# jgsimard/big-dreamer

Measured on AMD Instinct MI355X. Metric: latent transitions/sec (RSSM + imagination) at batch=50 chunk=50 H=15, higher is better.
Workload: dtype f32

## Files before the change

big_dreamer_amd/_cabi.py:

```python
from __future__ import annotations

import ctypes as C
import os

import torch

_HERE = os.path.dirname(os.path.abspath(__file__))
LIB_PATH = os.environ.get("BD_LIB") or os.path.join(_HERE, "libbigdreamer_hip.so")

if not os.path.exists(LIB_PATH):
    raise ImportError(
        f"{LIB_PATH} is missing: the MI355X HIP extension has not been built "
        "(run `python -c 'import __graft_entry__ as g; g.build()'`). There is no CPU fallback.")

lib = C.CDLL(LIB_PATH)

BD_MAX_LAYERS = 6
ACT_NONE, ACT_ELU, ACT_ELU_GRAD = 0, 1, 2
ACT_RELU, ACT_RELU_GRAD, ACT_TANH, ACT_TANH_GRAD = 3, 4, 5, 6
CNN_ACTS = {"ELU": (ACT_ELU, ACT_ELU_GRAD), "ReLU": (ACT_RELU, ACT_RELU_GRAD), "Tanh": (ACT_TANH, ACT_TANH_GRAD)}
GRAD_ACTS = (ACT_ELU_GRAD, ACT_RELU_GRAD, ACT_TANH_GRAD)
P = C.c_void_p
F32 = C.c_float
I32 = C.c_int
# ... 8 lines not shown


class MlpFwdArgs(C.Structure):
    _fields_ = [("M", I32), ("in0", P), ("ld0", I32), ("w0", I32), ("in1", P), ("ld1", I32), ("w1", I32),
                ("n_layers", I32), ("layer", Layer * BD_MAX_LAYERS), ("out", P), ("ldo", I32),
                ("gidx", P), ("gWT", P), ("gD", I32), ("gC", I32)]


class LayerBwd(C.Structure):
    _fields_ = [("wt", P), ("saved", P), ("N", I32), ("K", I32), ("act", I32), ("dpre", P)]


class MlpBwdArgs(C.Structure):
    _fields_ = [("M", I32), ("dout", P), ("lddo", I32), ("dout_scale", F32), ("n_layers", I32),
                ("layer", LayerBwd * BD_MAX_LAYERS), ("din0", P), ("ld0", I32), ("w0", I32),
                ("din1", P), ("ld1", I32), ("w1", I32), ("accumulate", I32), ("form_M", I32)]


BD_HEAD_HIDDEN = 4


class ImgHead(C.Structure):
    _fields_ = [("w", P * BD_HEAD_HIDDEN), ("wt", P * BD_HEAD_HIDDEN), ("b", P * BD_HEAD_HIDDEN),
                ("w_out", P), ("b_out", P), ("dout", P), ("out", P)]


class ImgHeadsArgs(C.Structure):
    _fields_ = [("M", I32), ("F", I32), ("Hd", I32), ("x", P), ("head", ImgHead * 2), ("dx", P)]


BD_RNG_MAX_TENSORS = 6
BD_RNG_NORMAL, BD_RNG_EXPONENTIAL, BD_RNG_UNIFORM = 0, 1, 2


class RngTensor(C.Structure):
    _fields_ = [("p", P), ("count", C.c_size_t), ("kind", I32), ("stream_id", C.c_uint)]


class RngFillArgs(C.Structure):
    _fields_ = [("n", I32), ("seed", C.c_ulonglong), ("step", C.c_ulonglong), ("t", RngTensor * BD_RNG_MAX_TENSORS)]


class WgradDesc(C.Structure):
# ... 170 lines not shown
    "bd_gemm_nt": (I32, [P, I32, P, I32, P, I32, I32, I32, I32, I32, P]),
    "bd_categorical_head_forward": (I32, [P, P, I32, I32, I32, P, P, P]),
    "bd_categorical_head_backward": (I32, [P, P, I32, I32, I32, P, P]),
    "bd_kl_categorical_forward": (I32, [P, P, I32, I32, I32, F32, I32, P, I32, P, P]),
    "bd_kl_categorical_backward": (I32, [P, P, I32, I32, I32, F32, F32, F32, F32, P, I32, P, P, P]),
    "bd_plan_rollout": (I32, [C.POINTER(PlanArgs), P]),
    "bd_cem_refit": (I32, [P, I32, P, I32, I32, I32, I32, I32, P, P, P]),
    "bd_plan_rollout_cat": (I32, [C.POINTER(PlanCatArgs), P]),
    "bd_act_step_supported": (I32, [I32, I32, I32, I32, I32, I32]),
    "bd_act_step": (I32, [C.POINTER(ActArgs), P]),
    "bd_act_step_cat_supported": (I32, [I32] * 10),
    "bd_act_step_cat": (I32, [C.POINTER(ActCatArgs), P]),
    "bd_lambda_return_backward": (I32, [P, F32, I32, I32, F32, F32, P, P, P]),
    "bd_img_heads_supported": (I32, [I32, I32]),
    "bd_img_heads_fwd_bwd": (I32, [C.POINTER(ImgHeadsArgs), P]),
    "bd_actor_reinforce": (I32, [P, P, P, P, P, P, P, I32, I32, I32, F32, F32, F32, I32, P, P, I32, P, P]),
    "bd_actor_reinforce_cat": (I32, [P, P, P, P, P, P, I32, I32, I32, F32, F32, F32, I32, P, P, I32, P, P]),
    "bd_normal_nll": (I32, [P, I32, P, I32, I32, I32, F32, P, I32, P, I32, P, P]),
    "bd_bernoulli_nll": (I32, [P, P, C.c_size_t, F32, P, P, I32, P, P]),
    "bd_kl_forward": (I32, [P, P, P, P, I32, I32, F32, I32, P, I32, P, P]),
    "bd_kl_backward": (I32, [P, P, P, P, I32, I32, F32, F32, F32, F32, P, I32, P, P, P, P, P]),
    "bd_sum": (I32, [P, C.c_size_t, P, I32, P, P]),
    "bd_sumsq": (I32, [P, C.c_size_t, P, I32, P, P]),
    "bd_adam_step": (I32, [P, P, P, P, C.c_size_t, F32, F32, F32, F32, F32, I32, F32, P, I32, P]),
    "bd_polyak": (I32, [P, P, C.c_size_t, F32, P]),
    "bd_replay_gather": (I32, [P, P, I32, I32, P, P]),
    "bd_replay_gather_pixels": (I32, [P, P, I32, I32, I32, P, P, P]),
    "bd_replay_gather_pixels_rng": (I32, [P, P, I32, I32, I32, C.c_ulonglong, C.c_ulonglong, P, P]),
    "bd_replay_append": (I32, [C.POINTER(ReplayAppendArgs), P]),
    "bd_reduce_ws_floats": (C.c_size_t, []),
# ... 45 lines not shown
```

big_dreamer_amd/csrc/mlp.hip:

```cpp
#include "bd_device.h"
#include "bd_host.h"
#include <stdlib.h>

namespace bd {

template <bool ANY>
__device__ __forceinline__ floatx4 chain_act4(int act, floatx4 x) {
    if constexpr (ANY) return act_apply4(act, x);
    floatx4 v = x;
    if (act) {
#pragma unroll
        for (int r = 0; r < 4; ++r) v[r] = elu(x[r]);
    }
    return v;
}
template <bool ANY>
__device__ __forceinline__ float chain_grad(int act, float y) {
    if constexpr (ANY) return act_grad_from_out(act, y);
    return elu_grad_from_out(y);
}

template <int RT, bool ANY>
__global__ __launch_bounds__(kThreads) void mlp_fwd_kernel(bd_mlp_fwd_args a, int KbA, int KbB) {
    extern __shared__ __attribute__((aligned(16))) float smem[];
// ... 130 lines not shown
        float* t = cur; cur = nxt; nxt = t;
    }
    if (a.din0 != nullptr || a.din1 != nullptr) {
        const bd_layer_bwd L = a.layer[0];
        const Seg segs[1] = {{cur, L.wt, cdiv(L.N, 16)}};
        tile_linear_pre<RT, 1, true>(segs, nullptr, L.K, NoPre{}, [&](int rt, int nb, floatx4 acc, NoPreVal) {
            const int ln = bd_tid() & 63, col0 = nb * 16 + 4 * (ln >> 4);
            const int grow = row0 + rt * 16 + (ln & 15);
            if (grow >= a.M) return;
#pragma unroll
            for (int r = 0; r < 4; ++r) {
                const int col = col0 + r;
                float* p = nullptr;
                if (col < a.w0) { if (a.din0) p = a.din0 + (size_t)grow * a.ld0 + col; }
                else if (col < a.w0 + a.w1) { if (a.din1) p = a.din1 + (size_t)grow * a.ld1 + (col - a.w0); }
                if (p) *p = a.accumulate ? *p + acc[r] : acc[r];
            }
        }, scratch);
    }
}

#ifdef BD_STAMPS
__device__ unsigned long long g_tallstamps[64];
#define TALL_STAMP(slot)                                                                                         \
    do {                                                                                                         \
        if (blockIdx.x == 0 && threadIdx.x == 0 && (slot) < 64) g_tallstamps[slot] = __builtin_amdgcn_s_memtime(); \
    } while (0)
#else
#define TALL_STAMP(slot)
#endif

template <int RT, bool ANY>
__global__ __launch_bounds__(kThreads) __attribute__((amdgpu_waves_per_eu(3, 3))) void mlp_fwd_tall_kernel(bd_mlp_fwd_args a) {
// ... 270 lines not shown
    bool any = false;
    for (int l = a->n_layers - 1, j = 0; l >= 0; --l, ++j) {
        const bd_layer_bwd& L = a->layer[l];
        any = any || (L.act != BD_ACT_NONE && L.act != BD_ACT_ELU);
        BD_REQUIRE(L.N > 0 && L.K > 0, "bd_mlp_backward: layer %d has bad dims", l);
        BD_REQUIRE(L.act == BD_ACT_NONE || act_is_forward(L.act), "bd_mlp_backward: layer %d has unknown activation code %d", l, L.act);
        BD_REQUIRE(!L.act || L.saved, "bd_mlp_backward: layer %d needs its saved output", l);
        BD_REQUIRE(l == 0 ? (!want_din || L.wt) : (L.wt != nullptr), "bd_mlp_backward: layer %d needs packed W^T", l);
        BD_REQUIRE(l == 0 || a->layer[l - 1].N == L.K, "bd_mlp_backward: layer %d K mismatch", l);
        int& kb = (j & 1) ? KbB : KbA;
        kb = cdiv(L.N, 16) > kb ? cdiv(L.N, 16) : kb;
    }
    if (want_din) BD_REQUIRE(a->w0 + a->w1 == a->layer[0].K, "bd_mlp_backward: din widths != K of layer 0");
    BD_REQUIRE(a->form_M >= 0, "bd_mlp_backward: bad form_M");
    const int Mf = a->form_M > 0 ? a->form_M : a->M;
    if (tall_enabled() && cdiv(Mf, 16) >= (tall_mode == 2 ? 1 : kTallMinTiles)) {
        bool ok = true;
        size_t widest = (size_t)(a->ld0 > a->ld1 ? a->ld0 : a->ld1);
        auto al16 = [](const void* q) { return (reinterpret_cast<uintptr_t>(q) & 15) == 0; };
        for (int l = a->n_layers - 1; l >= 1; --l) {
            const bd_layer_bwd& P = a->layer[l - 1];
            ok = ok && tall_shape_ok(a->layer[l].K, kTallRT) && (P.N & 3) == 0 && al16(P.saved) && al16(P.dpre);
            widest = (size_t)a->layer[l].K > widest ? (size_t)a->layer[l].K : widest;
        }
        ok = ok && (size_t)a->M * widest < ((size_t)1 << 31);
        int kb = KbA > KbB ? KbA : KbB;
        if (want_din) kb = cdiv(a->layer[0].N, 16) > kb ? cdiv(a->layer[0].N, 16) : kb;
        if (ok && any) return launch_tall(mlp_bwd_tall_kernel<kTallRT, true>, "bd_mlp_backward(tall)", a->M, kb, (hipStream_t)stream, *a);
        if (ok) return launch_tall(mlp_bwd_tall_kernel<kTallRT, false>, "bd_mlp_backward(tall)", a->M, kb, (hipStream_t)stream, *a);
    }
    const int rt = pick_rt(Mf, KbA, KbB);
    if (any) {
        if (rt == 2) return launch_chain(mlp_bwd_kernel<2, true>, "bd_mlp_backward", a->M, 2, KbA, KbB, (hipStream_t)stream, *a);
        return launch_chain(mlp_bwd_kernel<1, true>, "bd_mlp_backward", a->M, 1, KbA, KbB, (hipStream_t)stream, *a);
    }
    if (rt == 2) return launch_chain(mlp_bwd_kernel<2, false>, "bd_mlp_backward", a->M, 2, KbA, KbB, (hipStream_t)stream, *a);
    return launch_chain(mlp_bwd_kernel<1, false>, "bd_mlp_backward", a->M, 1, KbA, KbB, (hipStream_t)stream, *a);
}

}
```

big_dreamer_amd/engine.py:

```python
from __future__ import annotations

import collections.abc
import ctypes as C
import math
import os
import weakref
from typing import Dict, List, Optional, Tuple

import numpy as np
import torch

from . import _cabi as cabi
from .parallel import DataParallel
from .params import ParamGroup, _adam_state_dict, _load_adam_state_dict
from .synth import CNN_ACTIVATIONS, DENSE_LAYERS, MODEL_MODULES, Dims, model_modules, param_shapes

lib = cabi.lib
ptr = cabi.ptr

DEFAULT_HP = dict(
    kl_balance=0.8, kl_loss_weight=0.1, free_nats=3.0, grad_clip_norm=100.0, discount=0.995, disclam=0.95,
    model_learning_rate=2e-4, actor_learning_rate=4e-5, value_learning_rate=1e-4, adam_epsilon=1e-5,
    weight_decay=1e-6, entropy_weight=1e-5, polyak_avg=1.0, min_std_dev=0.1, discount_weight=5.0,
    gradient_mixing=-1,
# ... 193 lines not shown
        self._mod_group.update(actor="actor", critic="critic", critic_target="critic_target")
        if params is not None:
            self.load_params(params)
        self.scalars = torch.zeros(N_SLOTS, dtype=torch.float32, device=self.dev)
        self.red_ws = torch.zeros(int(lib.bd_reduce_ws_floats()), dtype=torch.float32, device=self.dev)
        self._wgrad_ws = torch.zeros(1, dtype=torch.float32, device=self.dev)
        self._wgrad_ws_side = torch.zeros(1, dtype=torch.float32, device=self.dev)
        self._wgrad_ws_early = torch.zeros(1, dtype=torch.float32, device=self.dev)
        self.red_ws_side = torch.zeros(int(lib.bd_reduce_ws_floats()), dtype=torch.float32, device=self.dev)
        self._wbatch = {"model": WgradBatch(self, "model"), "model_early": WgradBatch(self, "model_early", "_wgrad_ws_early"),
                        "actor": WgradBatch(self, "actor", "_wgrad_ws_bh"),
                        "critic": WgradBatch(self, "critic", "_wgrad_ws_side")}
        self._side = _engine_stream(self.dev, "side", int(os.environ.get("BD_SIDE_PRIO", "0")))
        self.heads_fused = (os.environ.get("BD_HEADS_FUSED", "1") != "0" and not self.d.categorical
                            and bool(lib.bd_img_heads_supported(self.d.Be + self.d.S, self.d.Hd)))
        self._s_early = _engine_stream(self.dev, "early", int(os.environ.get("BD_EARLY_PRIO", "0")))
        self.bh_chunks = _parse_bh_chunks(os.environ.get("BD_BH_CHUNKS", ""))
        self.bh_chunks_bwd = os.environ.get("BD_BH_CHUNKS_BWD", "0") == "1"
        self._s_ov = self._side
        self.pipeline = os.environ.get("BD_PIPELINE", "1") != "0"
        self._s_wm = _engine_stream(self.dev, "wm", int(os.environ.get("BD_WM_PRIO", "-1")))
        bh_prio = int(os.environ.get("BD_BH_PRIO", "0" if self.pixel else "-1"))
        self._s_bh = _engine_stream(self.dev, "bh", bh_prio)
        self._ev_bh_wm_free: Optional[torch.cuda.Event] = None
        self._bh_plan_used: Optional[Tuple[int, ...]] = None
        self._ev_bh_done: List[Optional[torch.cuda.Event]] = [None, None]
        self._ev_cr_done: List[Optional[torch.cuda.Event]] = [None, None]
        shared_comm = not all(g in self.dp.groups for g in ("model", "actor", "critic"))
        self.defer_opt = (world_size > 1 and shared_comm) or os.environ.get("BD_DEFER_OPT", "0") == "1"
        if os.environ.get("BD_FORCE_DP", "0") == "1" and torch.distributed.is_initialized():
# ... 215 lines not shown
    def mlp_forward(self, M, in0, ld0, w0, layers, saves, out, ldo, in1=None, ld1=0, w1=0, raw_packs=False,
                    gather=None) -> None:
        a = cabi.MlpFwdArgs()
        a.M, a.in0, a.ld0, a.w0 = M, ptr(in0), ld0, w0
        a.in1, a.ld1, a.w1 = ptr(in1), ld1, w1
        if gather is not None:
            a.gidx, a.gWT, a.gD, a.gC = ptr(gather[0]), ptr(gather[1]), gather[2], gather[3]
        a.n_layers = len(layers)
        for i, (key, bias, N, K, act) in enumerate(layers):
            a.layer[i] = cabi.Layer(ptr(key if raw_packs else self.pk[key]), ptr(bias), N, K, act,
                                    ptr(saves[i]) if saves else None)
        a.out, a.ldo = ptr(out), ldo
        cabi.check(lib.bd_mlp_forward(C.byref(a), cabi.stream()))

    def mlp_backward(self, M, dout, lddo, layers, saves, dpres, din0=None, ld0=0, w0=0, din1=None, ld1=0, w1=0,
                     accumulate=False, dout_scale=1.0, raw_packs=False, form_M=0) -> None:
        a = cabi.MlpBwdArgs()
        a.M, a.dout, a.lddo, a.dout_scale, a.form_M = M, ptr(dout), lddo, dout_scale, form_M
        a.n_layers = len(layers)
        for i, (key, _bias, N, K, act) in enumerate(layers):
            wt = key if raw_packs else self.pk.get(key + ".T")
            a.layer[i] = cabi.LayerBwd(ptr(wt) if wt is not None else None,
                                       ptr(saves[i]) if (saves and saves[i] is not None) else None, N, K, act,
                                       ptr(dpres[i]) if (dpres and dpres[i] is not None) else None)
        a.din0, a.ld0, a.w0 = ptr(din0), ld0, w0
        a.din1, a.ld1, a.w1 = ptr(din1), ld1, w1
        a.accumulate = int(accumulate)
        cabi.check(lib.bd_mlp_backward(C.byref(a), cabi.stream()))

    def wgrad(self, dpre, ldp, act, lda, M, N, K, dW, ldw, db=None, accumulate=False) -> None:
        need = int(lib.bd_wgrad_ws_floats(M, N, K))
        if self._wgrad_ws.numel() < need:
            self._wgrad_ws = torch.zeros(need, dtype=torch.float32, device=self.dev)
        cabi.check(lib.bd_wgrad(ptr(dpre), ldp, ptr(act), lda, M, N, K, ptr(dW), ldw, ptr(db), int(accumulate),
                                ptr(self._wgrad_ws), self._wgrad_ws.numel(), cabi.stream()))

    def _dense_wgrads(self, batch: "WgradBatch", mod: str, M: int, dpres, inp, ld_in, saves, sizes) -> None:
        for l in range(len(sizes) - 1):
            act, lda = (inp, ld_in) if l == 0 else (saves[l - 1], sizes[l])
            batch.add(dpres[l], sizes[l + 1], act, lda, M, sizes[l + 1], sizes[l],
                      self.G(mod, f"model.{2 * l}.weight"), sizes[l], self.G(mod, f"model.{2 * l}.bias"))

# ... 703 lines not shown
        N = T * B
        F = d.Be + d.S
        W = self.world_size
        st = cabi.stream()
        sc, ws = ptr(self.scalars), ptr(self.red_ws)

        obs_t = obs[1:].reshape(N, d.O)
        with self.span("encoder_fwd"):
            emb, pre_emb = self.encode_pixels(obs[1:].reshape(N, 3, 64, 64)) if self.pixel else self.encode(obs_t, N)
        init_belief = self.buf("init_belief", B, d.Be).zero_()
        init_state = self.buf("init_state", B, d.S).zero_()
        feat, qm, qs = self.observe(actions[:-1], nonterm[:-1], pre_emb, noise["obs_post"], init_belief, init_state, T, B,
                                    feat_tag=feat_tag)
        cat = d.categorical
        sidx = self._buf[feat_tag + "sidx"] if cat else None
        with self.span("wm_heads_fwd"):
            _, pm, ps = self.prior_head(feat, N, None if cat else noise.get("obs_prior"))
            if self.pixel:
                om_out, om_acts, om_layers = self.conv.decode(feat).view(N, d.O), None, None
                obs_t = self.conv.acts_enc[0].view(N, d.O)
            else:
                om_out, om_acts, om_layers = self.dense_forward("observation_model", "obs", "om", feat, F, N, d.O,
                                                                sidx=sidx)
            rw_out, rw_acts, rw_layers = self.dense_forward("reward_model", "rew", "rw", feat, F, N, 1, sidx=sidx)

        inv_rows = self.dp.mean_grad_scale(N)
        dc_state = None
        if d.use_discount:
            dc_out, dc_acts, dc_layers = self.dense_forward("discount_model", "dsc", "dc", feat, F, N, 1, sidx=sidx)
            d_dc = self.buf("d_dc_out", N, 1)
            cabi.check(lib.bd_bernoulli_nll(ptr(dc_out), ptr(nonterm[:-1]), N, hp["discount_weight"] * inv_rows, ptr(d_dc), sc,
                                            SLOT_DISC, ws, st))
            dc_state = (d_dc, dc_acts, dc_layers)
        d_om, d_rw = self.buf("d_om_out", N, d.O), self.buf("d_rw_out", N, 1)
        cabi.check(lib.bd_normal_nll(ptr(om_out), d.O, ptr(obs_t), d.O, N, d.O, inv_rows, ptr(d_om), d.O, sc, SLOT_OBS, ws, st))
        cabi.check(lib.bd_normal_nll(ptr(rw_out), 1, ptr(rewards[:-1]), 1, N, 1, inv_rows, ptr(d_rw), 1, sc, SLOT_REW, ws, st))
        sum_form = int(hp["kl_balance"] == -1)
        kl_n = d.cat_D if cat else d.S
        if cat:
            cabi.check(lib.bd_kl_categorical_forward(ptr(qm), ptr(pm), N, d.cat_D, d.cat_C, hp["free_nats"], sum_form, sc,
                                                     SLOT_KL, ws, st))
        else:
            cabi.check(lib.bd_kl_forward(ptr(qm), ptr(qs), ptr(pm), ptr(ps), N, d.S, hp["free_nats"], sum_form, sc, SLOT_KL,
                                         ws, st))
        if W > 1 and not sum_form:
            self._kl_local = self.scalars[SLOT_KL:SLOT_KL + 1].clone()
            self._allreduce(self.scalars[SLOT_KL:SLOT_KL + 1], "model")
        kl_inv = 1.0 / (N * kl_n * W) if not sum_form else 1.0 / (N * W)
        kl_w = hp["kl_loss_weight"] * (1.0 / W if sum_form else 1.0)
        if cat:
            dqm, dpm = self.buf("dql", N, d.S), self.buf("dpl", N, d.S)
            cabi.check(lib.bd_kl_categorical_backward(ptr(qm), ptr(pm), N, d.cat_D, d.cat_C, hp["free_nats"], hp["kl_balance"],
                                                      kl_w, kl_inv, sc, SLOT_KL, ptr(dqm), ptr(dpm), st))
        else:
            dqm, dqs = self.buf("dqm", N, d.S), self.buf("dqs", N, d.S)
            dpm, dps = self.buf("dpm", N, d.S), self.buf("dps", N, d.S)
            cabi.check(lib.bd_kl_backward(ptr(qm), ptr(qs), ptr(pm), ptr(ps), N, d.S, hp["free_nats"], hp["kl_balance"],
                                          kl_w, kl_inv, sc, SLOT_KL, ptr(dqm), ptr(dqs), ptr(dpm), ptr(dps), st))

        dfeat = self.buf("dfeat", N, F)
        rw_dpre = [self.buf(f"rw_dpre{l}", N, d.Hd) for l in range(DENSE_LAYERS)] + [d_rw]
        if self.pixel:
            self.mlp_backward(N, d_rw, 1, rw_layers, rw_acts + [None], rw_dpre[:-1] + [None], din0=dfeat, ld0=F, w0=F)
            with self.span("decoder_bwd"):
                self.conv.backward_decoder(d_om.view(N, 64, 64, 3), feat, dfeat, self._wbatch["model_early"])
                self._s_early.wait_stream(torch.cuda.current_stream())
                with torch.cuda.stream(self._s_early):
                    self._wbatch["model_early"].run()
        else:
            om_dpre = [self.buf(f"om_dpre{l}", N, d.Hd) for l in range(DENSE_LAYERS)] + [d_om]
            self.mlp_backward(N, d_om, d.O, om_layers, om_acts + [None], om_dpre[:-1] + [None], din0=dfeat, ld0=F, w0=F)
            self.mlp_backward(N, d_rw, 1, rw_layers, rw_acts + [None], rw_dpre[:-1] + [None], din0=dfeat, ld0=F, w0=F,
                              accumulate=True)
        dc_dpre = None
        if dc_state is not None:
            d_dc, dc_acts, dc_layers = dc_state
            dc_dpre = [self.buf(f"dc_dpre{l}", N, d.Hd) for l in range(DENSE_LAYERS)] + [d_dc]
            self.mlp_backward(N, d_dc, 1, dc_layers, dc_acts + [None], dc_dpre[:-1] + [None], din0=dfeat, ld0=F, w0=F,
                              accumulate=True)
        self._dc_wgrad = (dc_dpre, dc_state[1]) if dc_state is not None else None
        p_out, p_hid = self._buf["p_out"], self._buf["p_hid"]
        HO = d.head_out
        d_p_hid = self.buf("d_p_hid", N, d.Hd)
        if cat:
            d_p_out = dpm
        else:
            d_p_out = self.buf("d_p_out", N, HO)
            cabi.check(lib.bd_gauss_head_backward(ptr(p_out), None, None, ptr(dpm), ptr(dps), N, d.S, ptr(d_p_out), st))
        p_layers = [("p1", None, d.Hd, d.Be, cabi.ACT_ELU), ("p2", None, HO, d.Hd, cabi.ACT_NONE)]
        self.mlp_backward(N, d_p_out, HO, p_layers, [p_hid, None], [d_p_hid, None], din0=dfeat, ld0=F, w0=d.Be,
                          accumulate=True)
        d_e, d_gi, d_gh, d_q1, d_q2 = self._observe_backward(T, B, nonterm[:-1], noise["obs_post"], feat)
        self._dynamics_tail(batch, emb, obs_t, feat, init_belief, actions, d_e, d_gi, d_gh, d_q1, d_q2, d_p_hid, d_p_out,
                            p_hid, rw_dpre, rw_acts, om_dpre if (not self.pixel) else None,
                            om_acts if (not self.pixel) else None, N, B, F)
        return feat

    def _observe_backward(self, T: int, B: int, nonterm, eps_post, feat):
        d, pk, buf = self.d, self.pk, self._buf
        N = T * B
        if d.categorical:
            b = cabi.ObserveCatBwdArgs()
            b.D, b.C = d.cat_D, d.cat_C
            b.wt_q2 = ptr(pk["q2.T"])
            b.post_logits, b.dpost_logits = ptr(buf["post_logits"]), ptr(buf["dql"])
            scan, scan_cluster = lib.bd_observe_cat_backward, lib.bd_observe_cat_backward_cluster
# ... 51 lines not shown
        dense_sizes = lambda i, o: [i] + [d.Hd] * DENSE_LAYERS + [o]
        self._dense_wgrads(wb, "reward_model", N, rw_dpre, feat, F, rw_acts, dense_sizes(F, 1))
        if self._dc_wgrad is not None:
            self._dense_wgrads(wb, "discount_model", N, self._dc_wgrad[0], feat, F, self._dc_wgrad[1], dense_sizes(F, 1))
        if not self.pixel:
            self._dense_wgrads(wb, "observation_model", N, om_dpre, feat, F, om_acts, dense_sizes(F, d.O))
            self._dense_wgrads(wb, "encoder", N, enc_dpre, obs_t, d.O, enc_acts, dense_sizes(d.O, d.E))
        with self.span("wgrad_model"):
            wb.run()
        if self.pixel:
            torch.cuda.current_stream().wait_stream(self._s_early)
        if self.pipeline and self._ev_bh_wm_free is not None:
            torch.cuda.current_stream().wait_event(self._ev_bh_wm_free)
        with self.span("opt_model"):
            self.optimizer_step("model", SLOT_GN_MODEL, hp["model_learning_rate"])

    def img_heads_fused(self, M: int, x, d_r, d_v, r_out, v_out, dx) -> None:
        d = self.d
        a = cabi.ImgHeadsArgs()
        a.M, a.F, a.Hd, a.x, a.dx = M, d.Be + d.S, d.Hd, ptr(x), ptr(dx)
        for h, (mod, prefix, dout, out) in enumerate((("reward_model", "rew", d_r, r_out),
                                                      ("critic_target", "tgt", d_v, v_out))):
            H = a.head[h]
            for l in range(DENSE_LAYERS):
                H.w[l], H.wt[l] = ptr(self.pk[f"{prefix}{l}"]), ptr(self.pk[f"{prefix}{l}.T"])
                H.b[l] = ptr(self.W(mod, f"model.{2 * l}.bias"))
            H.w_out = ptr(self.W(mod, f"model.{2 * DENSE_LAYERS}.weight"))
            H.b_out = ptr(self.W(mod, f"model.{2 * DENSE_LAYERS}.bias"))
            H.dout, H.out = ptr(dout), ptr(out)
        cabi.check(lib.bd_img_heads_fwd_bwd(C.byref(a), cabi.stream()))
# ... 293 lines not shown
```

include/bigdreamer_hip.h:

```cpp
#ifndef BIGDREAMER_HIP_H
#define BIGDREAMER_HIP_H

#include <stddef.h>
#include <stdint.h>

#ifdef __cplusplus
extern "C" {
#endif

#define BD_MAX_LAYERS 6
#define BD_ACT_NONE 0
#define BD_ACT_ELU 1
#define BD_ACT_ELU_GRAD 2
#define BD_ACT_RELU 3
#define BD_ACT_RELU_GRAD 4
#define BD_ACT_TANH 5
#define BD_ACT_TANH_GRAD 6

const char* bd_last_error(void);
int bd_version(void);

typedef struct {
    const float* src;
    float* dst;
// ... 30 lines not shown
    int N, K;
    int act;
    float* dpre;
} bd_layer_bwd;

typedef struct {
    int M;
    const float* dout; int lddo;
    float dout_scale;
    int n_layers;
    bd_layer_bwd layer[BD_MAX_LAYERS];
    float* din0; int ld0, w0;
    float* din1; int ld1, w1;
    int accumulate;
    int form_M;
} bd_mlp_bwd_args;
int bd_mlp_backward(const bd_mlp_bwd_args* a, void* stream);

int bd_mlp_set_tall(int mode);

size_t bd_wgrad_ws_floats(int M, int N, int K);
int bd_wgrad(const float* dpre, int ldp, const float* act, int lda, int M, int N, int K,
             float* dW, int ldw, float* db, int accumulate, float* ws, size_t ws_floats, void* stream);

typedef struct {
    const float* dpre; int ldp;
    const float* act1; int lda1; int M1;
    const float* act2; int lda2;
    int M, N, K;
    float* dW; int ldw;
// ... 166 lines not shown
    const float* wt[BD_HEAD_HIDDEN];
    const float* b[BD_HEAD_HIDDEN];
    const float* w_out;
    const float* b_out;
    const float* dout;
    float* out;
} bd_img_head;
typedef struct {
    int M, F, Hd;
    const float* x;
    bd_img_head head[2];
    float* dx;
} bd_img_heads_args;
int bd_img_heads_supported(int F, int Hd);
int bd_img_heads_fwd_bwd(const bd_img_heads_args* a, void* stream);

int bd_actor_reinforce(const float* eps_action, const float* act_us, const float* act_stats, const float* returns,
                       const float* base0, const float* value, const float* weight, int Hm, int N, int A, float rho,
                       float grad_scale, float dentropy, int write, float* d_actor_out, float* scalars, int slot, float* ws,
                       void* stream);
int bd_actor_reinforce_cat(const float* action, const float* act_stats, const float* returns, const float* base0,
                           const float* value, const float* weight, int Hm, int N, int A, float rho, float grad_scale,
                           float dentropy, int write, float* d_actor_out, float* scalars, int slot, float* ws,
                           void* stream);

#define BD_RNG_MAX_TENSORS 6
#define BD_RNG_NORMAL 0
#define BD_RNG_EXPONENTIAL 1
#define BD_RNG_UNIFORM 2
typedef struct {
// ... 246 lines not shown
```

Before: 13.46 million.

## Fuse world-model obs, reward and prior heads into one forward+backward kernel

Adds a wm_heads kernel that runs the observation and reward decoder MLPs (forward, loss gradient, backward to the input) and the belief prior head (forward and Gaussian parameterisation) as three block-row chains in a single launch, keeping activations in LDS. The reward head's input gradient goes to a side buffer and is folded into dfeat by a new din0_add path in the next accumulating mlp_backward, replacing separate forward, NLL-gradient and backward launches. This cuts launches and round-trips of activations through global memory. In exchange it adds LDS pressure, only 16-row tiles per block, and a constraint that the tall backward form cannot take the add path.

```diff
diff --git a/big_dreamer_amd/_cabi.py b/big_dreamer_amd/_cabi.py
--- a/big_dreamer_amd/_cabi.py
+++ b/big_dreamer_amd/_cabi.py
@@ -46,7 +46,8 @@
 class MlpBwdArgs(C.Structure):
     _fields_ = [("M", I32), ("dout", P), ("lddo", I32), ("dout_scale", F32), ("n_layers", I32),
                 ("layer", LayerBwd * BD_MAX_LAYERS), ("din0", P), ("ld0", I32), ("w0", I32),
-                ("din1", P), ("ld1", I32), ("w1", I32), ("accumulate", I32), ("form_M", I32)]
+                ("din1", P), ("ld1", I32), ("w1", I32), ("accumulate", I32), ("form_M", I32),
+                ("din0_add", P), ("ld_add", I32), ("w_add", I32)]
 
 
 BD_HEAD_HIDDEN = 4
@@ -59,6 +60,20 @@
 
 class ImgHeadsArgs(C.Structure):
     _fields_ = [("M", I32), ("F", I32), ("Hd", I32), ("x", P), ("head", ImgHead * 2), ("dx", P)]
+
+
+class WmLayer(C.Structure):
+    _fields_ = [("w", P), ("wt", P), ("bias", P), ("N", I32), ("K", I32), ("save", P), ("dpre", P)]
+
+
+class WmChain(C.Structure):
+    _fields_ = [("n_layers", I32), ("w_in", I32), ("layer", WmLayer * BD_MAX_LAYERS), ("out", P), ("ldo", I32),
+                ("target", P), ("ldt", I32), ("grad_scale", F32), ("dx", P), ("lddx", I32)]
+
+
+class WmHeadsArgs(C.Structure):
+    _fields_ = [("M", I32), ("S", I32), ("x", P), ("ldx", I32), ("chain", WmChain * 3), ("eps", P), ("min_std", F32),
+                ("mean", P), ("std", P), ("state", P)]
 
 
 BD_RNG_MAX_TENSORS = 6
@@ -259,6 +274,8 @@
     "bd_lambda_return_backward": (I32, [P, F32, I32, I32, F32, F32, P, P, P]),
     "bd_img_heads_supported": (I32, [I32, I32]),
     "bd_img_heads_fwd_bwd": (I32, [C.POINTER(ImgHeadsArgs), P]),
+    "bd_wm_heads_supported": (I32, [I32, I32, I32, I32, I32]),
+    "bd_wm_heads_fwd_bwd": (I32, [C.POINTER(WmHeadsArgs), P]),
     "bd_actor_reinforce": (I32, [P, P, P, P, P, P, P, I32, I32, I32, F32, F32, F32, I32, P, P, I32, P, P]),
     "bd_actor_reinforce_cat": (I32, [P, P, P, P, P, P, I32, I32, I32, F32, F32, F32, I32, P, P, I32, P, P]),
     "bd_normal_nll": (I32, [P, I32, P, I32, I32, I32, F32, P, I32, P, I32, P, P]),
diff --git a/big_dreamer_amd/csrc/mlp.hip b/big_dreamer_amd/csrc/mlp.hip
--- a/big_dreamer_amd/csrc/mlp.hip
+++ b/big_dreamer_amd/csrc/mlp.hip
@@ -168,9 +168,24 @@
                 float* p = nullptr;
                 if (col < a.w0) { if (a.din0) p = a.din0 + (size_t)grow * a.ld0 + col; }
                 else if (col < a.w0 + a.w1) { if (a.din1) p = a.din1 + (size_t)grow * a.ld1 + (col - a.w0); }
-                if (p) *p = a.accumulate ? *p + acc[r] : acc[r];
+                if (!p) continue;
+                float o = acc[r];
+                if (a.accumulate) {
+                    float b = *p;
+                    if (a.din0_add && col < a.w0) b = b + a.din0_add[(size_t)grow * a.ld_add + col];
+                    o = b + acc[r];
+                }
+                *p = o;
             }
         }, scratch);
+        if (a.din0_add && a.w_add > a.w0) {
+            const int wt = a.w_add - a.w0;
+            for (int i = bd_tid(); i < 16 * RT * wt; i += blockDim.x) {
+                const int r = i / wt, col = a.w0 + (i - r * wt);
+                const int grow = row0 + r;
+                if (grow < a.M) a.din0[(size_t)grow * a.ld0 + col] += a.din0_add[(size_t)grow * a.ld_add + col];
+            }
+        }
     }
 }
 
@@ -471,6 +486,13 @@
     if (want_din) BD_REQUIRE(a->w0 + a->w1 == a->layer[0].K, "bd_mlp_backward: din widths != K of layer 0");
     BD_REQUIRE(a->form_M >= 0, "bd_mlp_backward: bad form_M");
     const int Mf = a->form_M > 0 ? a->form_M : a->M;
+    if (a->din0_add) {
+        BD_REQUIRE(a->accumulate == 1 && a->din0, "bd_mlp_backward: din0_add needs accumulate = 1 and din0");
+        BD_REQUIRE(a->w_add == 0 || (a->w_add >= a->w0 && a->din1 == nullptr && a->ld0 >= a->w_add),
+                   "bd_mlp_backward: w_add = %d needs w0 <= w_add <= ld0 and din1 = NULL", a->w_add);
+        BD_REQUIRE(a->ld_add >= (a->w_add > a->w0 ? a->w_add : a->w0), "bd_mlp_backward: ld_add = %d is smaller than the columns added",
+                   a->ld_add);
+    }
     if (tall_enabled() && cdiv(Mf, 16) >= (tall_mode == 2 ? 1 : kTallMinTiles)) {
         bool ok = true;
         size_t widest = (size_t)(a->ld0 > a->ld1 ? a->ld0 : a->ld1);
@@ -483,6 +505,7 @@
         ok = ok && (size_t)a->M * widest < ((size_t)1 << 31);
         int kb = KbA > KbB ? KbA : KbB;
         if (want_din) kb = cdiv(a->layer[0].N, 16) > kb ? cdiv(a->layer[0].N, 16) : kb;
+        if (ok) BD_REQUIRE(!a->din0_add, "bd_mlp_backward: din0_add is not taken by the tall form (%d rows pick it)", Mf);
         if (ok && any) return launch_tall(mlp_bwd_tall_kernel<kTallRT, true>, "bd_mlp_backward(tall)", a->M, kb, (hipStream_t)stream, *a);
         if (ok) return launch_tall(mlp_bwd_tall_kernel<kTallRT, false>, "bd_mlp_backward(tall)", a->M, kb, (hipStream_t)stream, *a);
     }
diff --git a/big_dreamer_amd/csrc/wm_heads.hip b/big_dreamer_amd/csrc/wm_heads.hip
--- /dev/null
+++ b/big_dreamer_amd/csrc/wm_heads.hip
@@ -0,0 +1,234 @@
+#include "bd_device.h"
+#include "bd_host.h"
+
+namespace bd {
+
+constexpr int kWmChains = 3;
+
+template <class CL>
+__device__ __forceinline__ bd_wm_layer wm_layer(const CL& l) {
+    bd_wm_layer r;
+    r.w = l.w; r.wt = l.wt; r.bias = l.bias; r.N = l.N; r.K = l.K; r.save = l.save; r.dpre = l.dpre;
+    return r;
+}
+
+__global__ __launch_bounds__(kThreads) void wm_heads_kernel(bd_wm_heads_args a, int KbA, int KbB) {
+    extern __shared__ __attribute__((aligned(16))) float smem[];
+    BD_KARGS(bd_wm_heads_args, ka);
+    const auto& C = ka->chain[blockIdx.y];
+    const int M = ka->M, row0 = blockIdx.x * 16, n = C.n_layers;
+    const bool loss = C.target != nullptr;
+    float* cur = smem;
+    float* nxt = smem + (size_t)KbA * kFragFloats;
+    float* scratch = nxt + (size_t)KbB * kFragFloats;
+    load_tile_concat<1>(cur, cdiv(C.w_in, 16), row0, M, ka->x, ka->ldx, C.w_in, nullptr, 0, 0);
+    lds_barrier();
+    auto al16 = [](const void* q) { return (reinterpret_cast<uintptr_t>(q) & 15) == 0; };
+    for (int l = 0; l < n; ++l) {
+        const bd_wm_layer L = wm_layer(C.layer[l]);
+        const bool last = (l == n - 1);
+        const int Kb = cdiv(L.K, 16);
+        float* out = C.out;
+        const float* target = C.target;
+        const int ldo = C.ldo, ldt = C.ldt;
+        const float gs = C.grad_scale;
+        const bool vec = (L.N & 3) == 0 && (last ? (!loss && (ldo & 3) == 0 && al16(out)) : al16(L.save));
+        const Seg seg[1] = {{cur, L.w, Kb}};
+        tile_linear_pre<1, 1, true>(
+            seg, L.bias, L.N,
+            [&](int, int nb) {
+                Pre4 p;
+                const int ln = bd_tid() & 63, col0 = nb * 16 + 4 * (ln >> 4);
+                const int grow = row0 + (ln & 15);
+#pragma unroll
+                for (int r = 0; r < 4; ++r)
+                    p.v[r] = (last && loss && grow < M && col0 + r < L.N) ? target[(size_t)grow * ldt + col0 + r] : 0.f;
+                return p;
+            },
+            [&](int, int nb, floatx4 acc, const Pre4& p) {
+                const int ln = bd_tid() & 63, col0 = nb * 16 + 4 * (ln >> 4);
+                const int grow = row0 + (ln & 15);
+                floatx4 v = acc, img;
+                if (!last) {
+#pragma unroll
+                    for (int r = 0; r < 4; ++r) v[r] = elu(acc[r]);
+                }
+                img = v;
+                if (last && loss) {
+#pragma unroll
+                    for (int r = 0; r < 4; ++r) img[r] = (grow < M && col0 + r < L.N) ? (v[r] - p.v[r]) * gs : 0.f;
+                }
+                *reinterpret_cast<floatx4*>(nxt + (nb * 64 + ln) * 4) = img;
+                if (grow < M && col0 < L.N) {
+                    if (vec) {
+                        if (last) *reinterpret_cast<floatx4*>(out + (size_t)grow * ldo + col0) = v;
+                        else *reinterpret_cast<floatx4*>(L.save + (size_t)grow * L.N + col0) = v;
+                    } else {
+#pragma unroll
+                        for (int r = 0; r < 4; ++r)
+                            if (col0 + r < L.N) {
+                                if (!last) L.save[(size_t)grow * L.N + col0 + r] = v[r];
+                                else {
+                                    out[(size_t)grow * ldo + col0 + r] = v[r];
+                                    if (loss) L.dpre[(size_t)grow * L.N + col0 + r] = img[r];
+                                }
+                            }
+                    }
+                }
+            },
+            scratch);
+        if (last && loss) __syncthreads();
+        else lds_barrier();
+        float* t = cur; cur = nxt; nxt = t;
+    }
+    if (!loss) {
+        const int S = ka->S;
+        const float* eps = ka->eps;
+        const float min_std = ka->min_std;
+        float* mean = ka->mean;
+        float* std = ka->std;
+        float* state = ka->state;
+        for (int i = bd_tid(); i < 16 * S; i += kThreads) {
+            const int row = i / S, c = i - row * S;
+            const int grow = row0 + row;
+            if (grow >= M) continue;
+            const size_t g = (size_t)grow * S + c;
+            const float m = cur[frag_idx(row, c)];
+            const float sd = softplusf(cur[frag_idx(row, S + c)]) + min_std;
+            mean[g] = m;
+            std[g] = sd;
+            if (state) state[g] = m + sd * eps[g];
+        }
+        return;
+    }
+    for (int l = n - 1; l >= 1; --l) {
+        const bd_wm_layer L = wm_layer(C.layer[l]);
+        const bd_wm_layer P = wm_layer(C.layer[l - 1]);
+        const int Kb = cdiv(L.N, 16);
+        const Seg segs[1] = {{cur, L.wt, Kb}};
+        const bool vec = (P.N & 3) == 0 && al16(P.save) && al16(P.dpre);
+        tile_linear_pre<1, 1, true>(
+            segs, nullptr, L.K,
+            [&](int, int nb) {
+                Pre4 p;
+                const int ln = bd_tid() & 63, col0 = nb * 16 + 4 * (ln >> 4);
+                const int grow = row0 + (ln & 15);
+                const bool in = grow < M && col0 < P.N;
+                if (in && vec) {
+                    const floatx4 t = *reinterpret_cast<const floatx4*>(P.save + (size_t)grow * P.N + col0);
+#pragma unroll
+                    for (int r = 0; r < 4; ++r) p.v[r] = t[r];
+                } else {
+#pragma unroll
+                    for (int r = 0; r < 4; ++r) p.v[r] = (in && col0 + r < P.N) ? P.save[(size_t)grow * P.N + col0 + r] : 1.f;
+                }
+                return p;
+            },
+            [&](int, int nb, floatx4 acc, const Pre4& p) {
+                const int ln = bd_tid() & 63, col0 = nb * 16 + 4 * (ln >> 4);
+                const int grow = row0 + (ln & 15);
+                floatx4 v = floatx4{0.f, 0.f, 0.f, 0.f};
+                if (grow < M && col0 < P.N) {
+#pragma unroll
+                    for (int r = 0; r < 4; ++r)
+                        if (col0 + r < P.N) v[r] = acc[r] * elu_grad_from_out(p.v[r]);
+                    if (vec) *reinterpret_cast<floatx4*>(P.dpre + (size_t)grow * P.N + col0) = v;
+                    else {
+#pragma unroll
+                        for (int r = 0; r < 4; ++r)
+                            if (col0 + r < P.N) P.dpre[(size_t)grow * P.N + col0 + r] = v[r];
+                    }
+                }
+                *reinterpret_cast<floatx4*>(nxt + (nb * 64 + ln) * 4) = v;
+            },
+            scratch);
+        lds_barrier();
+        float* t = cur; cur = nxt; nxt = t;
+    }
+    {
+        const bd_wm_layer L = wm_layer(C.layer[0]);
+        float* dx = C.dx;
+        const int lddx = C.lddx;
+        const Seg segs[1] = {{cur, L.wt, cdiv(L.N, 16)}};
+        tile_linear_pre<1, 1, true>(segs, nullptr, L.K, NoPre{}, [&](int, int nb, floatx4 acc, NoPreVal) {
+            const int ln = bd_tid() & 63, col0 = nb * 16 + 4 * (ln >> 4);
+            const int grow = row0 + (ln & 15);
+            if (grow >= M) return;
+#pragma unroll
+            for (int r = 0; r < 4; ++r)
+                if (col0 + r < L.K) dx[(size_t)grow * lddx + col0 + r] = acc[r];
+        }, scratch);
+    }
+}
+
+static void wm_plan_chain(const int* widths, int n, bool loss, int (&cap)[2]) {
+    int b = 0;
+    auto need = [&](int w) { cap[b] = cdiv(w, 16) > cap[b] ? cdiv(w, 16) : cap[b]; };
+    need(widths[0]);
+    for (int l = 1; l <= n; ++l) { b ^= 1; need(widths[l]); }
+    if (loss)
+        for (int l = n - 1; l >= 1; --l) { b ^= 1; need(widths[l]); }
+}
+
+static size_t wm_lds(const int (&cap)[2]) {
+    return ((size_t)(cap[0] + cap[1]) * kFragFloats + kSplitScratchFloats) * sizeof(float);
+}
+
+}
+
+extern "C" {
+
+int bd_wm_heads_supported(int Be, int S, int Hd, int O, int hidden) {
+    using namespace bd;
+    if (Be <= 0 || S <= 0 || Hd <= 0 || O <= 0 || hidden < 1 || hidden + 1 > BD_MAX_LAYERS) return 0;
+    int cap[2] = {0, 0}, w[BD_MAX_LAYERS + 1];
+    w[0] = Be + S;
+    for (int l = 1; l <= hidden; ++l) w[l] = Hd;
+    w[hidden + 1] = O > 1 ? O : 1;
+    wm_plan_chain(w, hidden + 1, true, cap);
+    const int p[3] = {Be, Hd, 2 * S};
+    wm_plan_chain(p, 2, false, cap);
+    return wm_lds(cap) <= (size_t)kMaxLds;
+}
+
+int bd_wm_heads_fwd_bwd(const bd_wm_heads_args* a, void* stream) {
+    using namespace bd;
+    BD_REQUIRE(a && a->M > 0 && a->S > 0 && a->x, "bd_wm_heads_fwd_bwd: bad M / S / x");
+    BD_REQUIRE(a->mean && a->std && (!a->state || a->eps), "bd_wm_heads_fwd_bwd: the prior needs mean and std, and eps for a sample");
+    int cap[2] = {0, 0};
+    for (int c = 0; c < kWmChains; ++c) {
+        const bd_wm_chain& C = a->chain[c];
+        const bool loss = c < kWmChains - 1;
+        BD_REQUIRE(C.n_layers >= 1 && C.n_layers <= BD_MAX_LAYERS, "bd_wm_heads_fwd_bwd: chain %d has bad n_layers", c);
+        BD_REQUIRE(C.w_in > 0 && a->ldx >= C.w_in, "bd_wm_heads_fwd_bwd: chain %d reads %d columns of x (ld %d)", c, C.w_in, a->ldx);
+        int w[BD_MAX_LAYERS + 1];
+        w[0] = C.w_in;
+        for (int l = 0; l < C.n_layers; ++l) {
+            const bd_wm_layer& L = C.layer[l];
+            const bool last = l == C.n_layers - 1;
+            BD_REQUIRE(L.N > 0 && L.K == w[l], "bd_wm_heads_fwd_bwd: chain %d layer %d has K=%d, expected %d", c, l, L.K, w[l]);
+            bool ok = L.w && (last || L.save);
+            if (loss) ok = ok && L.wt && L.dpre;
+            BD_REQUIRE(ok, "bd_wm_heads_fwd_bwd: chain %d layer %d is missing an operand", c, l);
+            w[l + 1] = L.N;
+        }
+        const int Nl = w[C.n_layers];
+        BD_REQUIRE(C.out && C.ldo >= Nl, "bd_wm_heads_fwd_bwd: chain %d has a bad output", c);
+        if (loss)
+            BD_REQUIRE(C.target && C.ldt >= Nl && C.dx && C.lddx >= C.w_in,
+                       "bd_wm_heads_fwd_bwd: chain %d is missing an operand (target / dx)", c);
+        else
+            BD_REQUIRE(!C.target && Nl == 2 * a->S, "bd_wm_heads_fwd_bwd: the prior chain ends in 2S = %d columns, got %d (no target)",
+                       2 * a->S, Nl);
+        wm_plan_chain(w, C.n_layers, loss, cap);
+    }
+    const size_t lds = wm_lds(cap);
+    BD_REQUIRE(lds <= (size_t)kMaxLds, "bd_wm_heads_fwd_bwd: widths not covered: the chain images need %zu B of LDS (> %d)", lds, kMaxLds);
+    if (lds > 64 * 1024 && allow_big_lds(wm_heads_kernel)) return -1;
+    hipLaunchKernelGGL(wm_heads_kernel, dim3(cdiv(a->M, 16), kWmChains), dim3(kThreads), lds, (hipStream_t)stream, *a,
+                       cap[0], cap[1]);
+    BD_CHECK_LAUNCH("bd_wm_heads_fwd_bwd");
+    return 0;
+}
+
+}
diff --git a/big_dreamer_amd/engine.py b/big_dreamer_amd/engine.py
--- a/big_dreamer_amd/engine.py
+++ b/big_dreamer_amd/engine.py
@@ -231,6 +231,8 @@
         self._side = _engine_stream(self.dev, "side", int(os.environ.get("BD_SIDE_PRIO", "0")))
         self.heads_fused = (os.environ.get("BD_HEADS_FUSED", "1") != "0" and not self.d.categorical
                             and bool(lib.bd_img_heads_supported(self.d.Be + self.d.S, self.d.Hd)))
+        self.wm_heads_fused = (os.environ.get("BD_WM_HEADS_FUSED", "1") != "0" and not self.d.categorical and not self.pixel
+                               and bool(lib.bd_wm_heads_supported(self.d.Be, self.d.S, self.d.Hd, self.d.O, DENSE_LAYERS)))
         self._s_early = _engine_stream(self.dev, "early", int(os.environ.get("BD_EARLY_PRIO", "0")))
         self.bh_chunks = _parse_bh_chunks(os.environ.get("BD_BH_CHUNKS", ""))
         self.bh_chunks_bwd = os.environ.get("BD_BH_CHUNKS_BWD", "0") == "1"
@@ -476,7 +478,7 @@
         cabi.check(lib.bd_mlp_forward(C.byref(a), cabi.stream()))
 
     def mlp_backward(self, M, dout, lddo, layers, saves, dpres, din0=None, ld0=0, w0=0, din1=None, ld1=0, w1=0,
-                     accumulate=False, dout_scale=1.0, raw_packs=False, form_M=0) -> None:
+                     accumulate=False, dout_scale=1.0, raw_packs=False, form_M=0, din0_add=None, ld_add=0, w_add=0) -> None:
         a = cabi.MlpBwdArgs()
         a.M, a.dout, a.lddo, a.dout_scale, a.form_M = M, ptr(dout), lddo, dout_scale, form_M
         a.n_layers = len(layers)
@@ -488,6 +490,7 @@
         a.din0, a.ld0, a.w0 = ptr(din0), ld0, w0
         a.din1, a.ld1, a.w1 = ptr(din1), ld1, w1
         a.accumulate = int(accumulate)
+        a.din0_add, a.ld_add, a.w_add = ptr(din0_add), ld_add, w_add
         cabi.check(lib.bd_mlp_backward(C.byref(a), cabi.stream()))
 
     def wgrad(self, dpre, ldp, act, lda, M, N, K, dW, ldw, db=None, accumulate=False) -> None:
@@ -1221,17 +1224,23 @@
                                     feat_tag=feat_tag)
         cat = d.categorical
         sidx = self._buf[feat_tag + "sidx"] if cat else None
+        inv_rows = self.dp.mean_grad_scale(N)
+        fused = self.wm_heads_fused and not cat and not self.pixel
+        dfeat = self.buf("dfeat", N, F)
         with self.span("wm_heads_fwd"):
-            _, pm, ps = self.prior_head(feat, N, None if cat else noise.get("obs_prior"))
-            if self.pixel:
-                om_out, om_acts, om_layers = self.conv.decode(feat).view(N, d.O), None, None
-                obs_t = self.conv.acts_enc[0].view(N, d.O)
+            if fused:
+                pm, ps, om, rw, dx_rw = self.wm_heads(feat, N, noise.get("obs_prior"), obs_t, rewards[:-1], inv_rows, dfeat)
+                (om_out, om_acts, om_layers, om_dpre), (rw_out, rw_acts, rw_layers, rw_dpre) = om, rw
             else:
-                om_out, om_acts, om_layers = self.dense_forward("observation_model", "obs", "om", feat, F, N, d.O,
-                                                                sidx=sidx)
-            rw_out, rw_acts, rw_layers = self.dense_forward("reward_model", "rew", "rw", feat, F, N, 1, sidx=sidx)
-
-        inv_rows = self.dp.mean_grad_scale(N)
+                _, pm, ps = self.prior_head(feat, N, None if cat else noise.get("obs_prior"))
+                if self.pixel:
+                    om_out, om_acts, om_layers = self.conv.decode(feat).view(N, d.O), None, None
+                    obs_t = self.conv.acts_enc[0].view(N, d.O)
+                else:
+                    om_out, om_acts, om_layers = self.dense_forward("observation_model", "obs", "om", feat, F, N, d.O,
+                                                                    sidx=sidx)
+                rw_out, rw_acts, rw_layers = self.dense_forward("reward_model", "rew", "rw", feat, F, N, 1, sidx=sidx)
+
         dc_state = None
         if d.use_discount:
             dc_out, dc_acts, dc_layers = self.dense_forward("discount_model", "dsc", "dc", feat, F, N, 1, sidx=sidx)
@@ -1240,8 +1249,10 @@
                                             SLOT_DISC, ws, st))
             dc_state = (d_dc, dc_acts, dc_layers)
         d_om, d_rw = self.buf("d_om_out", N, d.O), self.buf("d_rw_out", N, 1)
-        cabi.check(lib.bd_normal_nll(ptr(om_out), d.O, ptr(obs_t), d.O, N, d.O, inv_rows, ptr(d_om), d.O, sc, SLOT_OBS, ws, st))
-        cabi.check(lib.bd_normal_nll(ptr(rw_out), 1, ptr(rewards[:-1]), 1, N, 1, inv_rows, ptr(d_rw), 1, sc, SLOT_REW, ws, st))
+        cabi.check(lib.bd_normal_nll(ptr(om_out), d.O, ptr(obs_t), d.O, N, d.O, inv_rows, None if fused else ptr(d_om), d.O, sc,
+                                     SLOT_OBS, ws, st))
+        cabi.check(lib.bd_normal_nll(ptr(rw_out), 1, ptr(rewards[:-1]), 1, N, 1, inv_rows, None if fused else ptr(d_rw), 1, sc,
+                                     SLOT_REW, ws, st))
         sum_form = int(hp["kl_balance"] == -1)
         kl_n = d.cat_D if cat else d.S
         if cat:
@@ -1265,7 +1276,7 @@
             cabi.check(lib.bd_kl_backward(ptr(qm), ptr(qs), ptr(pm), ptr(ps), N, d.S, hp["free_nats"], hp["kl_balance"],
                                           kl_w, kl_inv, sc, SLOT_KL, ptr(dqm), ptr(dqs), ptr(dpm), ptr(dps), st))
 
-        dfeat = self.buf("dfeat", N, F)
+        add = dict(din0_add=dx_rw, ld_add=F, w_add=F) if fused else {}
         rw_dpre = [self.buf(f"rw_dpre{l}", N, d.Hd) for l in range(DENSE_LAYERS)] + [d_rw]
         if self.pixel:
             self.mlp_backward(N, d_rw, 1, rw_layers, rw_acts + [None], rw_dpre[:-1] + [None], din0=dfeat, ld0=F, w0=F)
@@ -1274,7 +1285,7 @@
                 self._s_early.wait_stream(torch.cuda.current_stream())
                 with torch.cuda.stream(self._s_early):
                     self._wbatch["model_early"].run()
-        else:
+        elif not fused:
             om_dpre = [self.buf(f"om_dpre{l}", N, d.Hd) for l in range(DENSE_LAYERS)] + [d_om]
             self.mlp_backward(N, d_om, d.O, om_layers, om_acts + [None], om_dpre[:-1] + [None], din0=dfeat, ld0=F, w0=F)
             self.mlp_backward(N, d_rw, 1, rw_layers, rw_acts + [None], rw_dpre[:-1] + [None], din0=dfeat, ld0=F, w0=F,
@@ -1284,7 +1295,8 @@
             d_dc, dc_acts, dc_layers = dc_state
             dc_dpre = [self.buf(f"dc_dpre{l}", N, d.Hd) for l in range(DENSE_LAYERS)] + [d_dc]
             self.mlp_backward(N, d_dc, 1, dc_layers, dc_acts + [None], dc_dpre[:-1] + [None], din0=dfeat, ld0=F, w0=F,
-                              accumulate=True)
+                              accumulate=True, **add)
+            add = {}
         self._dc_wgrad = (dc_dpre, dc_state[1]) if dc_state is not None else None
         p_out, p_hid = self._buf["p_out"], self._buf["p_hid"]
         HO = d.head_out
@@ -1296,7 +1308,7 @@
             cabi.check(lib.bd_gauss_head_backward(ptr(p_out), None, None, ptr(dpm), ptr(dps), N, d.S, ptr(d_p_out), st))
         p_layers = [("p1", None, d.Hd, d.Be, cabi.ACT_ELU), ("p2", None, HO, d.Hd, cabi.ACT_NONE)]
         self.mlp_backward(N, d_p_out, HO, p_layers, [p_hid, None], [d_p_hid, None], din0=dfeat, ld0=F, w0=d.Be,
-                          accumulate=True)
+                          accumulate=True, **add)
         d_e, d_gi, d_gh, d_q1, d_q2 = self._observe_backward(T, B, nonterm[:-1], noise["obs_post"], feat)
         self._dynamics_tail(batch, emb, obs_t, feat, init_belief, actions, d_e, d_gi, d_gh, d_q1, d_q2, d_p_hid, d_p_out,
                             p_hid, rw_dpre, rw_acts, om_dpre if (not self.pixel) else None,
@@ -1378,6 +1390,40 @@
             torch.cuda.current_stream().wait_event(self._ev_bh_wm_free)
         with self.span("opt_model"):
             self.optimizer_step("model", SLOT_GN_MODEL, hp["model_learning_rate"])
+
+    def wm_heads(self, feat, N: int, eps, obs_t, rew_t, grad_scale: float, dfeat):
+        d = self.d
+        F, HO = d.Be + d.S, d.head_out
+        a = cabi.WmHeadsArgs()
+        a.M, a.S, a.x, a.ldx = N, d.S, ptr(feat), F
+        heads = []
+        dx_rw = self.buf("dx_rw", N, F)
+        for c, (mod, prefix, tag, O, target, dx) in enumerate((("observation_model", "obs", "om", d.O, obs_t, dfeat),
+                                                               ("reward_model", "rew", "rw", 1, rew_t, dx_rw))):
+            layers = self._dense_spec(mod, prefix, F, O)
+            acts = [self.buf(f"{tag}_act{l}", N, d.Hd) for l in range(DENSE_LAYERS)]
+            dpre = [self.buf(f"{tag}_dpre{l}", N, d.Hd) for l in range(DENSE_LAYERS)] + [self.buf(f"d_{tag}_out", N, O)]
+            out = self.buf(f"{tag}_out", N, O)
+            ch = a.chain[c]
+            ch.n_layers, ch.w_in = len(layers), F
+            for l, (key, bias, Nl, Kl, _act) in enumerate(layers):
+                ch.layer[l] = cabi.WmLayer(ptr(self.pk[key]), ptr(self.pk[key + ".T"]), ptr(bias), Nl, Kl,
+                                           ptr(acts[l]) if l < DENSE_LAYERS else None, ptr(dpre[l]))
+            ch.out, ch.ldo, ch.target, ch.ldt, ch.grad_scale = ptr(out), O, ptr(target), O, grad_scale
+            ch.dx, ch.lddx = ptr(dx), F
+            heads.append((out, acts, layers, dpre))
+        tm = lambda n: self.W("transition_model", n)
+        hid, p_out = self.buf("p_hid", N, d.Hd), self.buf("p_out", N, HO)
+        ch = a.chain[2]
+        ch.n_layers, ch.w_in = 2, d.Be
+        ch.layer[0] = cabi.WmLayer(ptr(self.pk["p1"]), None, ptr(tm("belief_prior.model.0.bias")), d.Hd, d.Be, ptr(hid), None)
+        ch.layer[1] = cabi.WmLayer(ptr(self.pk["p2"]), None, ptr(tm("belief_prior.model.2.bias")), HO, d.Hd, None, None)
+        ch.out, ch.ldo = ptr(p_out), HO
+        pm, ps = self.buf("prior_mean", N, d.S), self.buf("prior_std", N, d.S)
+        pst = self.buf("prior_state", N, d.S) if eps is not None else None
+        a.eps, a.min_std, a.mean, a.std, a.state = ptr(eps), self.hp["min_std_dev"], ptr(pm), ptr(ps), ptr(pst)
+        cabi.check(lib.bd_wm_heads_fwd_bwd(C.byref(a), cabi.stream()))
+        return pm, ps, heads[0], heads[1], dx_rw
 
     def img_heads_fused(self, M: int, x, d_r, d_v, r_out, v_out, dx) -> None:
         d = self.d
diff --git a/include/bigdreamer_hip.h b/include/bigdreamer_hip.h
--- a/include/bigdreamer_hip.h
+++ b/include/bigdreamer_hip.h
@@ -68,6 +68,7 @@
     float* din1; int ld1, w1;
     int accumulate;
     int form_M;
+    const float* din0_add; int ld_add, w_add;
 } bd_mlp_bwd_args;
 int bd_mlp_backward(const bd_mlp_bwd_args* a, void* stream);
 
@@ -264,6 +265,33 @@
 } bd_img_heads_args;
 int bd_img_heads_supported(int F, int Hd);
 int bd_img_heads_fwd_bwd(const bd_img_heads_args* a, void* stream);
+
+typedef struct {
+    const float* w;
+    const float* wt;
+    const float* bias;
+    int N, K;
+    float* save;
+    float* dpre;
+} bd_wm_layer;
+typedef struct {
+    int n_layers, w_in;
+    bd_wm_layer layer[BD_MAX_LAYERS];
+    float* out; int ldo;
+    const float* target; int ldt;
+    float grad_scale;
+    float* dx; int lddx;
+} bd_wm_chain;
+typedef struct {
+    int M, S;
+    const float* x; int ldx;
+    bd_wm_chain chain[3];
+    const float* eps;
+    float min_std;
+    float* mean; float* std; float* state;
+} bd_wm_heads_args;
+int bd_wm_heads_supported(int Be, int S, int Hd, int O, int hidden);
+int bd_wm_heads_fwd_bwd(const bd_wm_heads_args* a, void* stream);
 
 int bd_actor_reinforce(const float* eps_action, const float* act_us, const float* act_stats, const float* returns,
                        const float* base0, const float* value, const float* weight, int Hm, int N, int A, float rho,
```

Measured after the change: 13.49 million (median of 6 runs). About the same (+0.2%).
